# carry4985/ORB_SLAM2_MAP

Measured on AMD Instinct MI355X. Metric: frames/sec ORB extract+match (640x480, 1000 feat), higher is better.
Workload: dtype u8; 1 GPU; C2: synthetic 640x480 RGB-D stream, 1000 features, 8 levels, extract + BF-Hamming match of consecutive frames; resident_frame_pool=1024, sequences=1, parallelism=1 sequence per GPU, schedule_name=best, extraction_parts=1

## Files before the change

orb_slam2_map_amd/csrc/extractor.hip:

```cpp
#include "common.h"

#include <atomic>
#include <chrono>
#include <thread>
#include <tuple>
#include <type_traits>
#include <utility>
#include "trig_base.h"
#include "pyramid_view.h"
#include "resize_tables.h"

#include <algorithm>
#include <cfloat>
#include <cmath>
#include <cstdlib>
#include <cstring>
#include <vector>

namespace orbgpu {

constexpr int EDGE = 19;
static_assert(EDGE == RS_EDGE, "resize_tables.h builds its tables for this border");
constexpr int BORDER0 = EDGE - 3;
constexpr int HALF_PATCH = 15;
// ... 1366 lines not shown
                    my_exp += c > 1;
                    k++;
                }
            }
            if (my_exp)
                atomicAdd(&s_nexp, my_exp);
            SYNC();

            QT_MARK(14)
            if (tid_ == 0) {
                s_n = n2;
                if (n2 >= N || n2 == n)
                    s_done = 1;
                else if (phase == 1 && n2 + 3 * s_nexp > N)
                    s_phase = 2;
            }
            SYNC();
        };
        if (n <= QT_SOLO_MAX) {
            if ((tid >> 6) == 0)
                node_sections(tid & 63, 64, [] { qt_wave_sync(); }, [](int *arr, int cnt) { return wave_excl_scan(arr, cnt); });
        } else
            node_sections(tid, nt, [] { __syncthreads(); }, [&](int *arr, int cnt) { return block_excl_scan(arr, cnt, s_tmp); });
        __syncthreads();
        done_cur = s_done;
        if (done_cur == 2)
            break;
        n_cur = s_n;
        phase_cur = s_phase;
        for (int i = tid; i < n_cur * 4; i += nt)
            S.ccnt_next[i] = 0;
        __syncthreads();
        const bool count_next = done_cur == 0;
        const bool last_pass = done_cur == 1;
        unsigned long long *best_next = reinterpret_cast<unsigned long long *>(S.ccnt_next);

        QT_MARK(15)
        for (int i0 = tid; i0 - tid < nkeys; i0 += QT_ILP * nt) {
            uint32_t key[QT_ILP];
            int nd[QT_ILP], nn[QT_ILP];
#pragma unroll
            for (int u = 0; u < QT_ILP; u++) {
                const int i = min(i0 + u * nt, nkeys - 1);
                key[u] = key_at(i);
                nd[u] = node_of(i, key[u]);
            }
#pragma unroll
            for (int u = 0; u < QT_ILP; u++)
                nn[u] = S.inE[nd[u]] ? S.cpos[nd[u] * 4 + quadrant_at(key[u], midA[nd[u]])] : S.opos[nd[u]];
#pragma unroll
            for (int u = 0; u < QT_ILP; u++) {
                const bool have = i0 + u * nt < nkeys;
                if (last_pass) {
                    if (have)
                        atomicMax(&best_next[nn[u]], best_of(key[u]));
                    continue;
                }
                if (have)
                    set_node(i0 + u * nt, nn[u]);
                if (count_next)
                    count_runs(S.ccnt_next, nn[u] * 4 + quadrant_at(key[u], midB[nn[u]]), have && cntB[nn[u]] > 1);
            }
        }
        __syncthreads();
        best_done = last_pass;
        labelled = labelled || !last_pass;
        {
            int *t = S.ccnt;
            S.ccnt = S.ccnt_next;
            S.ccnt_next = t;
        }
        {
            short4 *tb = bndA; bndA = bndB; bndB = tb;
            int *tc = cntA; cntA = cntB; cntB = tc;
            uint16_t *tr = creA; creA = creB; creB = tr;
            uint32_t *tm = midA; midA = midB; midB = tm;
        }
        __syncthreads();
    }

    QT_MARK(3)
    const int n = n_cur;
    unsigned long long *best = reinterpret_cast<unsigned long long *>(S.ccnt);
    if (!best_done) {
        for (int p = tid; p < n; p += nt)
            best[p] = 0ull;
        __syncthreads();
        for (int i0 = tid; i0 < nkeys; i0 += QT_ILP * nt) {
            uint32_t key[QT_ILP];
            int nd[QT_ILP];
#pragma unroll
            for (int u = 0; u < QT_ILP; u++) {
                const int i = min(i0 + u * nt, nkeys - 1);
                key[u] = key_at(i);
                nd[u] = node_of(i, key[u]);
            }
#pragma unroll
            for (int u = 0; u < QT_ILP; u++)
                if (i0 + u * nt < nkeys)
                    atomicMax(&best[nd[u]], best_of(key[u]));
        }
    }
    __syncthreads();
    uint32_t *osel = sel + (size_t)f * sel_cap_total + g.sel_off;
    const bool ok = done_cur != 2 && n <= g.sel_cap;
    for (int p = tid; p < n && ok; p += nt) {
        const unsigned long long b = best[p];
        const uint32_t yx = (uint32_t)((0xFFFFFFFFFFull - (b & 0xFFFFFFFFFFull)) & 0xFFFFFFull);
        osel[p] = (yx << 8) | (uint32_t)((b >> 40) - 1ull);
    }
    QT_MARK(4)
    if (tid == 0)
        nsel[(size_t)f * nlevels + level] = ok ? n : -1;
}

struct KpAux {
    int x, y, level;
    float angle;
    float ca, sb;
    int plane_off, pitch;
};

__device__ __forceinline__ float fast_atan2_deg(float y, float x)
{
    const float s = (float)(180 / 3.14159265358979323846);
    const float p1 = 0.9997878412794807f * s, p3 = -0.3258083974640975f * s;
    const float p5 = 0.1555786518463281f * s, p7 = -0.04432655554792128f * s;
    const float ax = fabsf(x), ay = fabsf(y);
    float a, c, c2;
    if (ax >= ay) {
        c = ay / (ax + (float)DBL_EPSILON);
        c2 = c * c;
        a = (((p7 * c2 + p5) * c2 + p3) * c2 + p1) * c;
    } else {
        c = ax / (ay + (float)DBL_EPSILON);
        c2 = c * c;
        a = 90.f - (((p7 * c2 + p5) * c2 + p3) * c2 + p1) * c;
    }
    if (x < 0)
        a = 180.f - a;
    if (y < 0)
        a = 360.f - a;
    return a;
}

struct UMax {
    int v[16];
};

constexpr int OR_ITERS = 4;
constexpr int OR_BATCH_MIN = 32;
constexpr int PYR_BATCH_MIN = 32;

__global__ __launch_bounds__(256) void k_orient(const uint8_t *__restrict__ pyr, size_t frame_pyr,
                                                const LevelGeom *__restrict__ geom, int nlevels,
                                                const uint32_t *__restrict__ sel, int sel_cap_total,
                                                const int *__restrict__ nsel, const uint32_t *__restrict__ orw,
                                                orbgpu_keypoint *__restrict__ kps, KpAux *__restrict__ aux,
                                                int cap, int *__restrict__ n_out, int iters, Src0 s0)
{
    __shared__ uint32_t W10[4 * 16 * 9], M01[4 * 16 * 9];
    __shared__ __align__(16) uint8_t stage[8][31 * 48];
    for (int i = threadIdx.x; i < 4 * 16 * 9; i += 256) {
        W10[i] = orw[i];
        M01[i] = orw[4 * 16 * 9 + i];
    }
    __syncthreads();

    const int hl = threadIdx.x & 31;
    int bx, f;
    xcd_frame_block(bx, f);
    f = serpentine(f);
    const int *ns = nsel + (size_t)f * nlevels;
    for (int it = 0; it < iters; it++) {
    const int slot = (bx * iters + it) * 8 + (threadIdx.x >> 5);
    int level = -1, j = 0, out_off = 0, total = 0, cnt_l = 0;
    bool bad = false;
    struct {
        int plane_off, pitch, sel_off, patch;
        float scale;
    } g = {0, 0, 0, 0, 1.f};
    for (int l = 0; l < nlevels; l++) {
        const int c = ns[l];
        if (c < 0)
            bad = true;
        const int so = geom[l].sel_off;
        if (slot >= so && slot < so + geom[l].sel_cap) {
            level = l;
            j = slot - so;
            out_off = total;
            cnt_l = c;
            g.plane_off = geom[l].plane_off;
            g.pitch = geom[l].pitch;
            g.sel_off = so;
            g.patch = geom[l].patch;
            g.scale = geom[l].scale;
        }
        total += max(c, 0);
    }
    if (slot == 0 && hl == 0)
        n_out[f] = bad ? -1 - total : (total > cap ? -1 - total : total);
    if (level < 0 || bad || total > cap || j >= cnt_l)
        continue;
    const uint32_t key = sel[(size_t)f * sel_cap_total + g.sel_off + j];
    const int x = key_x(key) + BORDER0, y = key_y(key) + BORDER0;
    const bool dir0 = s0.direct != 0 && level == 0;
    const int porg = dir0 ? 0 : EDGE, ppitch = dir0 ? (int)s0.pitch : g.pitch;
    const int xl = x + porg - HALF_PATCH;
    const int a = xl & 3;
    const int v = hl - HALF_PATCH;
    int m10 = 0, m01 = 0;
    {
        const uint8_t *base = (dir0 ? s0.p + (size_t)f * s0.frame_stride : pyr + (size_t)f * frame_pyr + g.plane_off) + (xl - a);
        struct __attribute__((packed, aligned(4))) Piece {
            uint32_t d[4];
        };
        const int lim = a == 2 ? 3 : (a == 3 ? 6 : -1);
        const uint8_t *rowbase = base + rowoff(y + porg - HALF_PATCH, ppitch);
        uint4 *pl = reinterpret_cast<uint4 *>(stage[threadIdx.x >> 5]);
        Piece pc[3];
#pragma unroll
        for (int k = 0; k < 2; k++) {
            const int q = hl + 32 * k, r = q >> 1, part = q & 1;
            if (q < 62)
                pc[k] = *reinterpret_cast<const Piece *>(rowbase + rowoff(r, ppitch) + part * 16);
        }
        const int r2 = HALF_PATCH - lim + hl;
        if (hl < 2 * lim + 1)
            pc[2] = *reinterpret_cast<const Piece *>(rowbase + rowoff(r2, ppitch) + 32);
#pragma unroll
        for (int k = 0; k < 2; k++) {
            const int q = hl + 32 * k;
            if (q < 62)
                pl[3 * (q >> 1) + (q & 1)] = make_uint4(pc[k].d[0], pc[k].d[1], pc[k].d[2], pc[k].d[3]);
        }
        if (hl < 2 * lim + 1)
            pl[3 * r2 + 2] = make_uint4(pc[2].d[0], pc[2].d[1], pc[2].d[2], pc[2].d[3]);
        __builtin_amdgcn_fence(__ATOMIC_RELEASE, "wavefront");
        __builtin_amdgcn_wave_barrier();
        __builtin_amdgcn_fence(__ATOMIC_ACQUIRE, "wavefront");
        if (hl < 31) {
            const int av = v < 0 ? -v : v;
            const uint32_t *row = reinterpret_cast<const uint32_t *>(stage[threadIdx.x >> 5]) + hl * 12;
            const uint32_t *w = &W10[(a * 16 + av) * 9], *m = &M01[(a * 16 + av) * 9];
            uint32_t sw = 0, sm = 0;
#pragma unroll
            for (int q = 0; q < 9; q++) {
                const uint32_t d = row[q];
                sw = __builtin_amdgcn_udot4(d, w[q], sw, false);
                sm = __builtin_amdgcn_udot4(d, m[q], sm, false);
            }
            m10 = (int)sw - 16 * (int)sm;
            m01 = v * (int)sm;
        }
        __builtin_amdgcn_fence(__ATOMIC_RELEASE, "wavefront");
        __builtin_amdgcn_wave_barrier();
    }
#pragma unroll
    for (int off = 16; off > 0; off >>= 1) {
        m10 += __shfl_xor(m10, off, 64);
        m01 += __shfl_xor(m01, off, 64);
    }
    if (hl == 0) {
        const float angle = fast_atan2_deg((float)m01, (float)m10);
        orbgpu_keypoint kp;
        kp.x = (float)x;
        kp.y = (float)y;
        if (level != 0) {
            kp.x *= g.scale;
            kp.y *= g.scale;
        }
        kp.size = (float)g.patch;
        kp.angle = angle;
        kp.response = (float)key_resp(key);
        kp.octave = level;
        kp.class_id = -1;
        kps[(size_t)f * cap + out_off + j] = kp;
        KpAux ax;
        ax.x = x + (dir0 ? BLUR0_OX - EDGE : 0);
        ax.y = y;
        ax.level = level;
        ax.plane_off = g.plane_off;
        ax.pitch = g.pitch;
        ax.angle = angle;
        aux[(size_t)f * cap + out_off + j] = ax;
    }
    }
}
__global__ __launch_bounds__(256) void k_trig(KpAux *__restrict__ aux, const int *__restrict__ n_out, int cap, TrigTable tt)
{
    const int f = blockIdx.y;
    const int i = blockIdx.x * 256 + threadIdx.x;
    if (i >= n_out[f])
        return;
    KpAux *a = aux + (size_t)f * cap + i;
    const float factorPI = (float)(3.14159265358979323846 / 180.f);
    const float angle = a->angle * factorPI;
    float c, s;
    orbgpu_trig_device(angle, tt, &c, &s);
    a->ca = c;
    a->sb = s;
}

constexpr int BLUR_ROWS = 30;

__device__ __forceinline__ void blur_hsum(uint32_t d0, uint32_t d1, uint32_t d2, uint32_t h[4])
{
#define W4(a, b, c, d) ((uint32_t)(a) | ((uint32_t)(b) << 8) | ((uint32_t)(c) << 16) | ((uint32_t)(d) << 24))
    h[0] = __builtin_amdgcn_udot4(d1, W4(55, 49, 34, 18), __builtin_amdgcn_udot4(d0, W4(0, 18, 34, 49), 0u, false), false);
    h[1] = __builtin_amdgcn_udot4(d2, W4(18, 0, 0, 0), __builtin_amdgcn_udot4(d1, W4(49, 55, 49, 34), __builtin_amdgcn_udot4(d0, W4(0, 0, 18, 34), 0u, false), false), false);
    h[2] = __builtin_amdgcn_udot4(d2, W4(34, 18, 0, 0), __builtin_amdgcn_udot4(d1, W4(34, 49, 55, 49), __builtin_amdgcn_udot4(d0, W4(0, 0, 0, 18), 0u, false), false), false);
    h[3] = __builtin_amdgcn_udot4(d2, W4(49, 34, 18, 0), __builtin_amdgcn_udot4(d1, W4(18, 34, 49, 55), 0u, false), false);
#undef W4
}

__device__ __forceinline__ uint32_t blur_vsum(const uint32_t A[4], const uint32_t C[4], const uint32_t E[4],
                                              const uint32_t F[4])
{
    const us2 K01 = {18, 34}, K23 = {49, 55}, K45 = {49, 34}, K6 = {0, 18};
    uint32_t sv[4];
#pragma unroll
    for (int p = 0; p < 4; p++) {
        uint32_t acc = __builtin_amdgcn_udot2(__builtin_bit_cast(us2, A[p]), K01, 32768u, false);
        acc = __builtin_amdgcn_udot2(__builtin_bit_cast(us2, C[p]), K23, acc, false);
        acc = __builtin_amdgcn_udot2(__builtin_bit_cast(us2, E[p]), K45, acc, false);
        sv[p] = __builtin_amdgcn_udot2(__builtin_bit_cast(us2, F[p]), K6, acc, false);
    }
    const us2 cap = {255, 255};
    const us2 lo = __builtin_elementwise_min(__builtin_bit_cast(us2, __builtin_amdgcn_perm(sv[1], sv[0], 0x07060302u)), cap);
    const us2 hi = __builtin_elementwise_min(__builtin_bit_cast(us2, __builtin_amdgcn_perm(sv[3], sv[2], 0x07060302u)), cap);
    return __builtin_amdgcn_perm(__builtin_bit_cast(uint32_t, hi), __builtin_bit_cast(uint32_t, lo), 0x06040200u);
}

__global__ __launch_bounds__(256) void k_blur(const uint8_t *__restrict__ pyr, uint8_t *__restrict__ blur,
                                               size_t frame_pyr, const LevelGeom *__restrict__ geom, StripGeom bg, int strip0)
{
    int bx, f;
    xcd_frame_block(bx, f);
    f = serpentine(f);
    const int strip = strip0 + bx * 256 + threadIdx.x;
    if (strip >= bg.first[bg.nlevels])
        return;
    int level = 0;
#pragma unroll
    for (int l = 1; l < ORBGPU_MAX_LEVELS; l++)
        level += (l < bg.nlevels && strip >= bg.first[l]) ? 1 : 0;
    const LevelGeom g = geom[level];
    const int local = strip - bg.first[level];
    const int sy = local / bg.nsx[level], sx = local - sy * bg.nsx[level];
    const int col = (4 + 2 * sx) * 4;
    const int y0 = sy * BLUR_ROWS;
    const int rows = min(BLUR_ROWS, g.h - y0);
    const uint8_t *fsrc = pyr + (size_t)f * frame_pyr;
    uint8_t *fdst = blur + (size_t)f * frame_pyr;
    const uint32_t pitch = (uint32_t)g.pitch;
    const uint32_t src0 = (uint32_t)g.plane_off + (uint32_t)(y0 + EDGE - 3) * pitch + (uint32_t)(col - 4);
    uint32_t soff = src0 + 6u * pitch;
    uint32_t doff = (uint32_t)g.plane_off + (uint32_t)(y0 + EDGE) * pitch + (uint32_t)col;
    struct __attribute__((packed, aligned(4))) Q4 {
        uint32_t d[4];
    };
    uint32_t p0[8], p1[8], p2[8], p3[8], p4[8], p5[8], hn[8];
    Q4 nx;
#define B8_HSUM(R, Q)                                                                                        \
    {                                                                                                        \
        blur_hsum(Q.d[0], Q.d[1], Q.d[2], R);                                                                \
        blur_hsum(Q.d[1], Q.d[2], Q.d[3], R + 4);                                                            \
    }
#define B8_PAIR(P, PREV, H)                                                                                  \
    _Pragma("unroll") for (int p = 0; p < 8; p++) P[p] = __builtin_amdgcn_alignbit(H[p], PREV[p], 16);
#define B8_LOAD(P, PREV, row)                                                                                \
    {                                                                                                        \
        const Q4 q = *reinterpret_cast<const Q4 *>(fsrc + (src0 + (uint32_t)(row) * pitch));                \
        B8_HSUM(hn, q)                                                                                       \
        B8_PAIR(P, PREV, hn)                                                                                 \
    }
#define B8_STEP(A, C, E, F, k)                                                                               \
    if ((k) < rows) {                                                                                        \
        B8_HSUM(hn, nx)                                                                                      \
        B8_PAIR(F, E, hn)                                                                                    \
        soff += pitch;                                                                                       \
        if ((k) + 1 < rows)                                                                                  \
            nx = *reinterpret_cast<const Q4 *>(fsrc + soff);                                                 \
        uint2 o;                                                                                             \
        o.x = blur_vsum(A, C, E, F);                                                                         \
        o.y = blur_vsum(A + 4, C + 4, E + 4, F + 4);                                                         \
        *reinterpret_cast<uint2 *>(fdst + doff) = o;                                                         \
        doff += pitch;                                                                                       \
    }
#pragma unroll
    for (int p = 0; p < 8; p++)
        p5[p] = 0;
    B8_LOAD(p5, p5, 0) B8_LOAD(p0, p5, 1) B8_LOAD(p1, p0, 2) B8_LOAD(p2, p1, 3) B8_LOAD(p3, p2, 4) B8_LOAD(p4, p3, 5)
    nx = *reinterpret_cast<const Q4 *>(fsrc + soff);
#pragma unroll 1
    for (int k = 0; k < BLUR_ROWS; k += 6) {
        B8_STEP(p0, p2, p4, p5, k)
        B8_STEP(p1, p3, p5, p0, k + 1)
        B8_STEP(p2, p4, p0, p1, k + 2)
        B8_STEP(p3, p5, p1, p2, k + 3)
        B8_STEP(p4, p0, p2, p3, k + 4)
        B8_STEP(p5, p1, p3, p4, k + 5)
    }
#undef B8_PAIR
#undef B8_STEP
#undef B8_LOAD
#undef B8_HSUM
}

__global__ __launch_bounds__(256) void k_blur0_direct(Src0 s0, uint8_t *__restrict__ blur, size_t frame_pyr,
                                                       const LevelGeom *__restrict__ geom)
{
    int bx, f;
    xcd_frame_block(bx, f);
    f = serpentine(f);
    const LevelGeom g = geom[0];
    const int nsx = g.w >> 3;
    const int strip = bx * 256 + threadIdx.x;
    const int sy = strip / nsx, sx = strip - sy * nsx;
    const int y0 = sy * BLUR_ROWS;
    if (y0 >= g.h)
        return;
    const int rows = min(BLUR_ROWS, g.h - y0);
    const bool first = sx == 0, last = sx == nsx - 1;
    const uint8_t *fsrc = s0.p + (size_t)f * s0.frame_stride + (first ? 0 : (last ? g.w - 16 : 8 * sx - 4));
    uint8_t *fdst = blur + (size_t)f * frame_pyr;
    const uint32_t pitch = (uint32_t)g.pitch;
    uint32_t doff = (uint32_t)g.plane_off + (uint32_t)(y0 + EDGE) * pitch + (uint32_t)(8 * sx + BLUR0_OX);
    struct __attribute__((packed, aligned(4))) Q4 {
        uint32_t d[4];
    };
    struct __attribute__((packed, aligned(4))) O2 {
        uint32_t d[2];
    };
    auto fetch = [&](int y) -> Q4 {
        const int ry = y < 0 ? -y : (y >= g.h ? 2 * g.h - 2 - y : y);
        return *reinterpret_cast<const Q4 *>(fsrc + __umul24((unsigned)ry, s0.pitch));
    };
    auto window = [&](const Q4 &q) -> Q4 {
        Q4 w;
        const uint32_t left = __builtin_amdgcn_perm(q.d[1], q.d[0], 0x01020304u);
// ... 759 lines not shown
    }
    if (which == 1)
        return;
    if (e->blur_geom.first[nl] > strip0)
        L.launch(k_blur, dim3((e->blur_geom.first[nl] - strip0 + 255) / 256, batch), dim3(256), 0, pyr, blur,
                           e->frame_pyr, dg, e->blur_geom, strip0);
}

static int launch_pipeline(orbgpu_extractor *e, const uint8_t *d_gray, int batch, int w, int h, size_t stride,
                           size_t frame_stride, orbgpu_keypoint *d_kps, uint8_t *d_desc, int cap, int *d_n_out,
                           Launcher &L)
{
    hipStream_t st = L.st;
    const int nl = e->nlevels;
    const LevelGeom *dg = e->d_geom.as<LevelGeom>();
    uint8_t *pyr = e->d_pyr.as<uint8_t>();
    uint8_t *blur = e->d_blur.as<uint8_t>();
    int rc = e->d_aux.reserve(sizeof(KpAux) * (size_t)cap * batch);
    if (rc != ORBGPU_OK)
        return rc;
    const bool rec = L.graph != nullptr;
    const bool prof = !rec && e->profiling && e->prof_calls < orbgpu_extractor::PROF_SLOTS;
    if (prof && e->ev.empty()) {
        e->ev.resize((size_t)orbgpu_extractor::PROF_SLOTS * 2 * ST_COUNT, nullptr);
        for (auto &x : e->ev)
            ORBGPU_HIP_TRY(hipEventCreate(&x));
    }
    hipEvent_t *evs = prof ? &e->ev[(size_t)e->prof_calls * 2 * ST_COUNT] : nullptr;
#define BEGIN(stage, s) if (prof && (stage) == 0) ORBGPU_HIP_TRY(hipEventRecord(evs[0], s))
#define END(stage, s)                                                          \
    {                                                                          \
        if (prof)                                                              \
            ORBGPU_HIP_TRY(hipEventRecord(evs[1 + (stage)], s));               \
        if (!rec && e->stage_signal[stage])                                    \
            ORBGPU_HIP_TRY(hipEventRecord(e->stage_signal[stage], s));         \
        if (!rec && e->pipe_signal[stage])                                     \
            ORBGPU_HIP_TRY(hipEventRecord(e->pipe_signal[stage], s));          \
    }
    const bool aligned4 = stride % 4 == 0 && frame_stride % 4 == 0 && (reinterpret_cast<uintptr_t>(d_gray) & 3) == 0;
    const bool direct = e->direct0_ok && !e->no_direct0 && aligned4 && batch >= e->direct0_min_batch;
    const Src0 s0{d_gray, frame_stride, (uint32_t)stride, direct ? 1 : 0};
    e->last_src = s0;
    e->level0_materialized = !direct;
    e->borders_materialized = !e->interior_resize;
    if (e->poison_pyramid) {
        int rcp = L.memset32(pyr, e->frame_pyr * batch, 0xA5);
        if (rcp == ORBGPU_OK)
            rcp = L.memset32(blur, e->frame_pyr * batch, 0xA5);
        if (rcp != ORBGPU_OK)
            return rcp;
    }
    BEGIN(ST_PYRAMID, st);
    const bool side_blur = e->concurrent_blur && !rec;
    Launcher Ls(e->side);
    const bool early_blur0 = side_blur && direct && !e->no_early_blur0;
    if (early_blur0) {
        ORBGPU_HIP_TRY(hipEventRecord(e->ev_fork0, st));
        ORBGPU_HIP_TRY(hipStreamWaitEvent(e->side, e->ev_fork0, 0));
        if (prof)
            ORBGPU_HIP_TRY(hipEventRecord(evs[ST_COUNT + 1], e->side));
        launch_blur(e, s0, batch, Ls, 1);
    }
    {
        if (!direct) {
            int rcb = materialize_level0(e, s0, batch, L);
            if (rcb != ORBGPU_OK)
                return rcb;
        }
        for (int l = 1; l < nl; l++) {
            const LevelGeom &gl = e->geom[l];
            dim3 gr((gl.pitch / 4 + 255) / 256, gl.h + 2 * EDGE, batch);
            const int ndw_l = (gl.pitch / 4) * (gl.h + 2 * EDGE);
            const int rows = batch >= PYR_BATCH_MIN || ndw_l >= 32768 ? PYR_ROWS : ndw_l >= 16384 ? PYR_ROWS / 2 : PYR_ROWS / 4;
            dim3 grf((resize_ndw(gl.w) * ((gl.h + rows - 1) / rows) + 255) / 256, batch);
            if (gl.rs_fast) {
                const bool dir1 = direct && l == 1;
                const int r8 = batch >= PYR_BATCH_MIN ? (dir1 ? e->r8_off_direct : e->r8_off[l]) : -1;
                if (r8 >= 0) {
                    dim3 gr8((resize_n8(gl.w) * ((gl.h + PYR_ROWS - 1) / PYR_ROWS) + 255) / 256, batch);
                    const bool shr = dir1 ? e->r8_share_direct : e->r8_share[l];
                    L.launch(dir1 ? (shr ? k_resize_fast<true, true, 8, true> : k_resize_fast<true, true, 8, false>)
                                  : (shr ? k_resize_fast<true, false, 8, true> : k_resize_fast<true, false, 8, false>), gr8, dim3(256), 0, pyr,
                             e->frame_pyr, dg, l, e->d_r8item.as<ResizeStrip>(), e->d_r8sel.as<uint4>(), e->d_r8wt.as<uint4>(),
                             e->d_yrow.as<YRow>(), r8, PYR_ROWS, s0);
                    continue;
                }
                auto kern = dir1 ? (rows == PYR_ROWS ? k_resize_fast<true, true, 4> : k_resize_fast<false, true, 4>)
                                 : (rows == PYR_ROWS ? k_resize_fast<true, false, 4> : k_resize_fast<false, false, 4>);
                L.launch(kern, grf, dim3(256), 0, pyr, e->frame_pyr, dg, l, e->d_rstrip.as<ResizeStrip>(),
                                   e->d_rsel.as<uint4>(), e->d_rwt.as<uint4>(), e->d_yrow.as<YRow>(),
                                   dir1 ? e->rs_off_direct : gl.rs_off, rows, s0);
            }
            else
                L.launch(k_resize_level, gr, dim3(256), 0, pyr, e->frame_pyr, dg, l,
                                   e->d_xtab.as<XTab>(), e->d_ytab.as<YTab>());
        }
    }
    END(ST_PYRAMID, st);
    BEGIN(ST_BLUR, st);
    if (side_blur) {
        ORBGPU_HIP_TRY(hipEventRecord(e->ev_fork, st));
        ORBGPU_HIP_TRY(hipStreamWaitEvent(e->side, e->ev_fork, 0));
        if (prof && !early_blur0)
            ORBGPU_HIP_TRY(hipEventRecord(evs[ST_COUNT + 1], e->side));
        launch_blur(e, s0, batch, Ls, early_blur0 ? 2 : 0);
        if (prof)
            ORBGPU_HIP_TRY(hipEventRecord(evs[ST_COUNT + 2], e->side));
        ORBGPU_HIP_TRY(hipEventRecord(e->ev_join, e->side));
    } else
        launch_blur(e, s0, batch, L);
    END(ST_BLUR, st);
    BEGIN(ST_FAST, st);
    if (e->counters_dirty) {
        int rcm = L.memset32(e->d_cellcnt.p, e->d_cellcnt.bytes & ~(size_t)3);
        if (rcm == ORBGPU_OK)
            rcm = L.memset32(e->d_qtaux.p, e->d_qtaux.bytes & ~(size_t)3);
        if (rcm != ORBGPU_OK)
            return rcm;
    }
    e->counters_dirty = true;
    {
        const int t_ini = std::max(e->prm.ini_th_fast, 1), t_min = std::max(e->prm.min_th_fast, 1);
        const DetectGeom &dgeo = direct ? e->det_geom_direct : e->det_geom;
        const int nwaves = (dgeo.first[nl] + FD_OWN - 1) / FD_OWN;
        L.launch(e->fast_early_out ? k_fast_detect<true> : k_fast_detect<false>, dim3((nwaves + 3) / 4, batch), dim3(256), 0, pyr, e->frame_pyr, dg,
                           dgeo, e->d_ctab.as<ColumnInfo>(), e->d_cells.as<CellDesc>(), (int)e->cells.size(),
                           e->d_slots.as<uint32_t>(), e->frame_slots, e->d_cellcnt.as<int>(), std::min(t_ini, t_min),
                           t_ini, e->fast_queue_cap, s0);
    }
    END(ST_FAST, st);
    BEGIN(ST_QUADTREE, st);
    if (batch >= QT_BATCH_MIN || e->force_batch_quadtree)
        L.launch(k_quadtree<false>, dim3(batch, nl), dim3(QT_THREADS_BATCH), e->qt_lds, dg,
                           e->d_cells.as<CellDesc>(), (int)e->cells.size(), e->d_slots.as<uint32_t>(), e->frame_slots,
                           e->d_cellcnt.as<int>(), e->d_dkey.as<uint32_t>(), e->d_dnode.as<uint16_t>(),
                           e->d_sel.as<uint32_t>(), e->sel_cap_total, e->d_nsel.as<int>(), e->d_ncand.as<int>(), nl,
                           e->ncap, std::max(e->prm.ini_th_fast, 1), 0, qt_dbg(), (int *)nullptr);
    else {
        if (e->qt_prefilter)
            L.launch(k_qt_prefilter, dim3(std::min((e->max_slots_level + QT_PRE_KEYS - 1) / QT_PRE_KEYS, QT_PRE_GRID), nl, batch), dim3(256), 0, dg, (int)e->cells.size(), e->d_slots.as<uint32_t>(), e->frame_slots, e->d_cellcnt.as<int>(),
                               e->d_dkey.as<uint32_t>(), e->d_qtaux.as<int>(), std::max(e->prm.ini_th_fast, 1));
        L.launch(k_quadtree<true>, dim3(batch, nl), dim3(w * h >= QT_LARGE_PIXELS ? QT_THREADS : QT_THREADS_SMALL), e->qt_lds + (size_t)e->qt_kcap * 6, dg,
                           e->d_cells.as<CellDesc>(), (int)e->cells.size(), e->d_slots.as<uint32_t>(), e->frame_slots,
                           e->d_cellcnt.as<int>(), e->d_dkey.as<uint32_t>(), e->d_dnode.as<uint16_t>(),
                           e->d_sel.as<uint32_t>(), e->sel_cap_total, e->d_nsel.as<int>(), e->d_ncand.as<int>(), nl,
                           e->ncap, std::max(e->prm.ini_th_fast, 1), e->qt_kcap, qt_dbg(),
                           e->qt_prefilter ? e->d_qtaux.as<int>() : (int *)nullptr);
    }
    if (!rec)
        ORBGPU_HIP_TRY(hipGetLastError());
    e->counters_dirty = false;
    END(ST_QUADTREE, st);
    BEGIN(ST_ORIENT, st);
    const int or_iters = batch >= OR_BATCH_MIN ? OR_ITERS : 1;
    L.launch(k_orient, dim3((e->sel_cap_total + 8 * or_iters - 1) / (8 * or_iters), batch), dim3(256), 0, pyr, e->frame_pyr, dg, nl,
                       e->d_sel.as<uint32_t>(), e->sel_cap_total, e->d_nsel.as<int>(),
                       reinterpret_cast<const uint32_t *>(e->d_pattern.as<uint8_t>() + 1024), d_kps,
                       e->d_aux.as<KpAux>(), cap, d_n_out, or_iters, s0);
    L.launch(k_trig, dim3((std::min(cap, e->max_kp) + 255) / 256, batch), dim3(256), 0,
                       e->d_aux.as<KpAux>(), d_n_out, cap, e->trig);
    END(ST_ORIENT, st);
    BEGIN(ST_DESCRIBE, st);
    if (side_blur)
        ORBGPU_HIP_TRY(hipStreamWaitEvent(st, e->ev_join, 0));
    L.launch(k_describe, dim3((std::min(cap, e->max_kp) + 7) / 8, batch), dim3(256), 0, blur,
                       e->frame_pyr, dg, e->d_aux.as<KpAux>(), d_n_out, cap, e->d_pattern.as<int8_t>(), d_desc);
    END(ST_DESCRIBE, st);
#undef BEGIN
#undef END
    if (!rec)
        ORBGPU_HIP_TRY(hipGetLastError());
    else if (L.err != hipSuccess) {
        set_error("recording the extraction graph: %s", hipGetErrorString(L.err));
        return ORBGPU_EHIP;
    }
    if (prof)
        e->prof_calls++;
    e->last_batch = batch;
    e->last_cap = cap;
    (void)w;
    (void)h;
    return ORBGPU_OK;
}

}

namespace orbgpu {

int extractor_pyramid_view(const orbgpu_extractor *e, PyramidView *v)
{
    ORBGPU_REQUIRE(e && v, "null argument");
    memset(v, 0, sizeof(*v));
    v->device_id = e->prm.device_id;
    v->nlevels = e->nlevels;
    v->scale_factor = e->prm.scale_factor;
    v->last_batch = (int)e->geom.size() == e->nlevels ? e->last_batch : 0;
    for (int l = 0; l < e->nlevels; l++) {
        v->scale[l] = e->scale[l];
        v->inv_scale[l] = e->inv_scale[l];
        if (v->last_batch > 0) {
            const LevelGeom &g = e->geom[l];
            v->w[l] = g.w;
            v->h[l] = g.h;
            v->pitch[l] = g.pitch;
            v->plane_off[l] = g.plane_off;
        }
    }
    v->pyr = e->d_pyr.as<uint8_t>();
    v->frame_pyr = e->frame_pyr;
    v->border = EDGE;
    v->direct = v->last_batch > 0 && e->last_src.direct ? 1 : 0;
    v->l0 = v->direct ? e->last_src.p : nullptr;
    v->l0_frame_stride = v->direct ? e->last_src.frame_stride : 0;
    v->l0_pitch = v->direct ? e->last_src.pitch : 0;
    v->scratch = &e->d_stereo;
    return ORBGPU_OK;
}

}

extern "C" {

int orbgpu_extractor_create(const orbgpu_extractor_params *p, orbgpu_extractor **out)
{
    std::lock_guard<std::mutex> lifecycle(orbgpu::lifecycle_mutex());
    ORBGPU_REQUIRE(p && out, "null argument");
    ORBGPU_REQUIRE(p->nlevels >= 1 && p->nlevels <= ORBGPU_MAX_LEVELS, "nlevels must be in [1,%d]", ORBGPU_MAX_LEVELS);
    ORBGPU_REQUIRE(p->nfeatures >= 1, "nfeatures must be positive");
    ORBGPU_REQUIRE(p->scale_factor > 1.0f, "scale_factor must be > 1");
    ORBGPU_REQUIRE(p->ini_th_fast >= 0 && p->ini_th_fast <= 255 && p->min_th_fast >= 0 && p->min_th_fast <= 255,
                   "FAST thresholds must be in [0,255]");
    int rc = select_device(p->device_id);
    if (rc != ORBGPU_OK)
        return rc;
    orbgpu_extractor *e = new (std::nothrow) orbgpu_extractor();
    if (!e) {
        set_error("out of host memory");
        return ORBGPU_ENOMEM;
    }
    e->prm = *p;
    if (e->prm.max_batch < 1)
        e->prm.max_batch = 1;
    e->force_batch_quadtree = getenv("ORBGPU_DEBUG_QT_BATCH") != nullptr;
    e->qt_no_prefilter = getenv("ORBGPU_DEBUG_QT_NOPRE") != nullptr;
    if (const char *q = getenv("ORBGPU_DEBUG_QT_KEYS"))
        e->qt_keys_hook = std::max(atoi(q), 0);
    e->no_direct0 = getenv("ORBGPU_DEBUG_NO_DIRECT0") != nullptr;
    e->poison_pyramid = getenv("ORBGPU_DEBUG_POISON_PYRAMID") != nullptr;
    e->no_early_blur0 = getenv("ORBGPU_DEBUG_NO_EARLY_BLUR0") != nullptr;
    if (const char *q = getenv("ORBGPU_DEBUG_DIRECT0_MIN"))
        e->direct0_min_batch = std::max(atoi(q), 1);
    if (const char *q = getenv("ORBGPU_FAST_EARLY_OUT"))
        e->fast_early_out = atoi(q) != 0;
    e->pinned_staging = getenv("ORBGPU_DEBUG_NO_PINNED") == nullptr;
    if (getenv("ORBGPU_DEBUG_NO_GRAPH"))
        e->graph_state = -1;
    if (const char *q = getenv("ORBGPU_DEBUG_FAST_QUEUE"))
        e->fast_queue_cap = std::min(std::max(atoi(q), 0), FD_QCAP);
    e->nlevels = p->nlevels;
    build_tables(e);
    hipError_t he = hipStreamCreateWithFlags(&e->stream, hipStreamNonBlocking);
    if (he != hipSuccess) {
        set_error("hipStreamCreate: %s", hipGetErrorString(he));
        delete e;
        return ORBGPU_EHIP;
    }
    rc = trig_table_for_device(p->device_id, &e->trig);
    if (rc != ORBGPU_OK) {
        (void)hipStreamDestroy(e->stream);
        delete e;
        return rc;
    }
    *out = e;
    return ORBGPU_OK;
}

int orbgpu_extractor_destroy(orbgpu_extractor *e)
{
    std::lock_guard<std::mutex> lifecycle(orbgpu::lifecycle_mutex());
    if (!e)
        return ORBGPU_OK;
    (void)hipSetDevice(e->prm.device_id);
    (void)hipDeviceSynchronize();
    DevBuf *bufs[] = {&e->d_geom, &e->d_cells, &e->d_xtab, &e->d_ytab, &e->d_yrow, &e->d_pattern, &e->d_rstrip, &e->d_rsel,
                      &e->d_rwt, &e->d_ctab, &e->d_bcol, &e->d_pyr,
                      &e->d_blur, &e->d_slots, &e->d_cellcnt, &e->d_dkey, &e->d_dnode, &e->d_sel, &e->d_nsel,
                      &e->d_ncand, &e->d_aux, &e->d_in, &e->d_kps, &e->d_desc, &e->d_nout, &e->d_dbg, &e->d_qtaux, &e->d_stereo};
    for (DevBuf *b : bufs)
        b->release();
    for (auto &x : e->ev)
        if (x)
            (void)hipEventDestroy(x);
    if (e->graph_exec)
        (void)hipGraphExecDestroy(e->graph_exec);
    if (e->graph)
        (void)hipGraphDestroy(e->graph);
    if (e->h_pin)
        (void)hipHostFree(e->h_pin);
    if (e->stream)
        (void)hipStreamDestroy(e->stream);
    if (e->side)
        (void)hipStreamDestroy(e->side);
    if (e->ev_fork)
        (void)hipEventDestroy(e->ev_fork);
    if (e->ev_fork0)
        (void)hipEventDestroy(e->ev_fork0);
    if (e->ev_join)
        (void)hipEventDestroy(e->ev_join);
    delete e;
    return ORBGPU_OK;
}

int orbgpu_extractor_get_levels(const orbgpu_extractor *e, int32_t *n)
// ... 576 lines not shown
```

Baseline: 297,500 frames/s.

## Template orient kernel, prefetch next patch, and fuse trig into orient for batches

The orientation kernel is templated on its iteration count. Keys and level geometry are loaded up front, the weight-table loads overlap the first patch fetch, and the global load for the next keypoint's patch is issued before the current one's moments are computed. For large batches the cosine/sine computation that k_trig did is folded into k_orient, which removes one kernel launch and a read-modify-write pass over the aux array. In exchange the kernel holds more registers and adds two block-wide syncs for the trig step.

Result: no change. 299,400 frames/s, median of 6 (+0.6%).

```diff
diff --git a/orb_slam2_map_amd/csrc/extractor.hip b/orb_slam2_map_amd/csrc/extractor.hip
--- a/orb_slam2_map_amd/csrc/extractor.hip
+++ b/orb_slam2_map_amd/csrc/extractor.hip
@@ -1542,141 +1542,223 @@
 constexpr int OR_BATCH_MIN = 32;
 constexpr int PYR_BATCH_MIN = 32;
 
+template <int ITERS, bool TRIG>
 __global__ __launch_bounds__(256) void k_orient(const uint8_t *__restrict__ pyr, size_t frame_pyr,
                                                 const LevelGeom *__restrict__ geom, int nlevels,
                                                 const uint32_t *__restrict__ sel, int sel_cap_total,
                                                 const int *__restrict__ nsel, const uint32_t *__restrict__ orw,
                                                 orbgpu_keypoint *__restrict__ kps, KpAux *__restrict__ aux,
-                                                int cap, int *__restrict__ n_out, int iters, Src0 s0)
-{
-    __shared__ uint32_t W10[4 * 16 * 9], M01[4 * 16 * 9];
+                                                int cap, int *__restrict__ n_out, Src0 s0, TrigTable tt)
+{
+    constexpr int NW = 4 * 16 * 9, NWK = (NW + 255) / 256;
+    __shared__ uint32_t W10[NW], M01[NW];
     __shared__ __align__(16) uint8_t stage[8][31 * 48];
-    for (int i = threadIdx.x; i < 4 * 16 * 9; i += 256) {
-        W10[i] = orw[i];
-        M01[i] = orw[4 * 16 * 9 + i];
-    }
-    __syncthreads();
-
+    uint32_t tw[NWK], tm[NWK];
+#pragma unroll
+    for (int k = 0; k < NWK; k++) {
+        const int i = min((int)threadIdx.x + 256 * k, NW - 1);
+        tw[k] = orw[i];
+        tm[k] = orw[NW + i];
+    }
     const int hl = threadIdx.x & 31;
+    const int hw = threadIdx.x >> 5;
+    const int half = threadIdx.x & 32;
     int bx, f;
     xcd_frame_block(bx, f);
     f = serpentine(f);
+    const int slot0 = bx * (ITERS * 8) + hw;
+    uint32_t key[ITERS];
+#pragma unroll
+    for (int it = 0; it < ITERS; it++)
+        key[it] = sel[(size_t)f * sel_cap_total + min(slot0 + 8 * it, sel_cap_total - 1)];
+    const LevelGeom *gl = geom + min(hl, nlevels - 1);
+    const int gl_plane = gl->plane_off, gl_pitch = gl->pitch, gl_patch = gl->patch;
+    const float gl_scale = gl->scale;
     const int *ns = nsel + (size_t)f * nlevels;
-    for (int it = 0; it < iters; it++) {
-    const int slot = (bx * iters + it) * 8 + (threadIdx.x >> 5);
-    int level = -1, j = 0, out_off = 0, total = 0, cnt_l = 0;
+    int lv[ITERS], oi[ITERS];
+#pragma unroll
+    for (int it = 0; it < ITERS; it++) {
+        lv[it] = -1;
+        oi[it] = 0;
+    }
+    int total = 0;
     bool bad = false;
-    struct {
-        int plane_off, pitch, sel_off, patch;
-        float scale;
-    } g = {0, 0, 0, 0, 1.f};
     for (int l = 0; l < nlevels; l++) {
         const int c = ns[l];
         if (c < 0)
             bad = true;
-        const int so = geom[l].sel_off;
-        if (slot >= so && slot < so + geom[l].sel_cap) {
-            level = l;
-            j = slot - so;
-            out_off = total;
-            cnt_l = c;
-            g.plane_off = geom[l].plane_off;
-            g.pitch = geom[l].pitch;
-            g.sel_off = so;
-            g.patch = geom[l].patch;
-            g.scale = geom[l].scale;
+        const int so = geom[l].sel_off, sc = geom[l].sel_cap;
+#pragma unroll
+        for (int it = 0; it < ITERS; it++) {
+            const int j = slot0 + 8 * it - so;
+            if (j >= 0 && j < sc) {
+                lv[it] = j < c ? l : -1;
+                oi[it] = total + j;
+            }
         }
         total += max(c, 0);
     }
-    if (slot == 0 && hl == 0)
+    if (bx == 0 && threadIdx.x == 0)
         n_out[f] = bad ? -1 - total : (total > cap ? -1 - total : total);
-    if (level < 0 || bad || total > cap || j >= cnt_l)
-        continue;
-    const uint32_t key = sel[(size_t)f * sel_cap_total + g.sel_off + j];
-    const int x = key_x(key) + BORDER0, y = key_y(key) + BORDER0;
-    const bool dir0 = s0.direct != 0 && level == 0;
-    const int porg = dir0 ? 0 : EDGE, ppitch = dir0 ? (int)s0.pitch : g.pitch;
-    const int xl = x + porg - HALF_PATCH;
-    const int a = xl & 3;
-    const int v = hl - HALF_PATCH;
-    int m10 = 0, m01 = 0;
-    {
-        const uint8_t *base = (dir0 ? s0.p + (size_t)f * s0.frame_stride : pyr + (size_t)f * frame_pyr + g.plane_off) + (xl - a);
-        struct __attribute__((packed, aligned(4))) Piece {
-            uint32_t d[4];
-        };
+    if (bad || total > cap) {
+#pragma unroll
+        for (int it = 0; it < ITERS; it++)
+            lv[it] = -1;
+    }
+
+    struct __attribute__((packed, aligned(4))) Piece {
+        uint32_t d[4];
+    };
+    Piece pc[3];
+    int al[ITERS] = {};
+    auto request = [&](int it) {
+        const int level = lv[it];
+        const bool dir0 = s0.direct != 0 && level == 0;
+        const int plane_off = __shfl(gl_plane, half + level, 64), pitch = __shfl(gl_pitch, half + level, 64);
+        const int x = key_x(key[it]) + BORDER0, y = key_y(key[it]) + BORDER0;
+        const int porg = dir0 ? 0 : EDGE, ppitch = dir0 ? (int)s0.pitch : pitch;
+        const int xl = x + porg - HALF_PATCH;
+        const int a = xl & 3;
+        al[it] = a;
+        const uint8_t *base = (dir0 ? s0.p + (size_t)f * s0.frame_stride : pyr + (size_t)f * frame_pyr + plane_off) + (xl - a);
         const int lim = a == 2 ? 3 : (a == 3 ? 6 : -1);
         const uint8_t *rowbase = base + rowoff(y + porg - HALF_PATCH, ppitch);
-        uint4 *pl = reinterpret_cast<uint4 *>(stage[threadIdx.x >> 5]);
-        Piece pc[3];
 #pragma unroll
         for (int k = 0; k < 2; k++) {
             const int q = hl + 32 * k, r = q >> 1, part = q & 1;
             if (q < 62)
                 pc[k] = *reinterpret_cast<const Piece *>(rowbase + rowoff(r, ppitch) + part * 16);
         }
-        const int r2 = HALF_PATCH - lim + hl;
         if (hl < 2 * lim + 1)
-            pc[2] = *reinterpret_cast<const Piece *>(rowbase + rowoff(r2, ppitch) + 32);
-#pragma unroll
-        for (int k = 0; k < 2; k++) {
-            const int q = hl + 32 * k;
-            if (q < 62)
-                pl[3 * (q >> 1) + (q & 1)] = make_uint4(pc[k].d[0], pc[k].d[1], pc[k].d[2], pc[k].d[3]);
-        }
-        if (hl < 2 * lim + 1)
-            pl[3 * r2 + 2] = make_uint4(pc[2].d[0], pc[2].d[1], pc[2].d[2], pc[2].d[3]);
+            pc[2] = *reinterpret_cast<const Piece *>(rowbase + rowoff(HALF_PATCH - lim + hl, ppitch) + 32);
+    };
+    if (lv[0] >= 0)
+        request(0);
+#pragma unroll
+    for (int k = 0; k < NWK; k++) {
+        const int i = threadIdx.x + 256 * k;
+        if (i < NW) {
+            W10[i] = tw[k];
+            M01[i] = tm[k];
+        }
+    }
+    __syncthreads();
+
+    const int v = hl - HALF_PATCH;
+    float ang[ITERS];
+#pragma unroll
+    for (int it = 0; it < ITERS; it++) {
+        ang[it] = 0.f;
+        const bool have = lv[it] >= 0;
+        const int a = al[it];
+        if (have) {
+            uint4 *pl = reinterpret_cast<uint4 *>(stage[hw]);
+            const int lim = a == 2 ? 3 : (a == 3 ? 6 : -1);
+#pragma unroll
+            for (int k = 0; k < 2; k++) {
+                const int q = hl + 32 * k;
+                if (q < 62)
+                    pl[3 * (q >> 1) + (q & 1)] = make_uint4(pc[k].d[0], pc[k].d[1], pc[k].d[2], pc[k].d[3]);
+            }
+            if (hl < 2 * lim + 1)
+                pl[3 * (HALF_PATCH - lim + hl) + 2] = make_uint4(pc[2].d[0], pc[2].d[1], pc[2].d[2], pc[2].d[3]);
+        }
         __builtin_amdgcn_fence(__ATOMIC_RELEASE, "wavefront");
         __builtin_amdgcn_wave_barrier();
         __builtin_amdgcn_fence(__ATOMIC_ACQUIRE, "wavefront");
-        if (hl < 31) {
-            const int av = v < 0 ? -v : v;
-            const uint32_t *row = reinterpret_cast<const uint32_t *>(stage[threadIdx.x >> 5]) + hl * 12;
-            const uint32_t *w = &W10[(a * 16 + av) * 9], *m = &M01[(a * 16 + av) * 9];
-            uint32_t sw = 0, sm = 0;
-#pragma unroll
-            for (int q = 0; q < 9; q++) {
-                const uint32_t d = row[q];
-                sw = __builtin_amdgcn_udot4(d, w[q], sw, false);
-                sm = __builtin_amdgcn_udot4(d, m[q], sm, false);
+        const int nx = it + 1 < ITERS ? it + 1 : it;
+        if (nx != it && lv[nx] >= 0)
+            request(nx);
+        if (have) {
+            int m10 = 0, m01 = 0;
+            if (hl < 31) {
+                const int av = v < 0 ? -v : v;
+                const uint32_t *row = reinterpret_cast<const uint32_t *>(stage[hw]) + hl * 12;
+                const uint32_t *w = &W10[(a * 16 + av) * 9], *m = &M01[(a * 16 + av) * 9];
+                uint32_t sw = 0, sm = 0;
+#pragma unroll
+                for (int q = 0; q < 9; q++) {
+                    const uint32_t d = row[q];
+                    sw = __builtin_amdgcn_udot4(d, w[q], sw, false);
+                    sm = __builtin_amdgcn_udot4(d, m[q], sm, false);
+                }
+                m10 = (int)sw - 16 * (int)sm;
+                m01 = v * (int)sm;
             }
-            m10 = (int)sw - 16 * (int)sm;
-            m01 = v * (int)sm;
+#pragma unroll
+            for (int off = 16; off > 0; off >>= 1) {
+                m10 += __shfl_xor(m10, off, 64);
+                m01 += __shfl_xor(m01, off, 64);
+            }
+            ang[it] = fast_atan2_deg((float)m01, (float)m10);
         }
         __builtin_amdgcn_fence(__ATOMIC_RELEASE, "wavefront");
         __builtin_amdgcn_wave_barrier();
     }
-#pragma unroll
-    for (int off = 16; off > 0; off >>= 1) {
-        m10 += __shfl_xor(m10, off, 64);
-        m01 += __shfl_xor(m01, off, 64);
-    }
-    if (hl == 0) {
-        const float angle = fast_atan2_deg((float)m01, (float)m10);
+
+    uint32_t mkey = 0;
+    int mlv = -1, moi = 0;
+    float angle = 0.f;
+#pragma unroll
+    for (int it = 0; it < ITERS; it++)
+        if (hl == it) {
+            mkey = key[it];
+            mlv = lv[it];
+            moi = oi[it];
+            angle = ang[it];
+        }
+    const int src = half + max(mlv, 0);
+    const int plane_off = __shfl(gl_plane, src, 64), pitch = __shfl(gl_pitch, src, 64), patch = __shfl(gl_patch, src, 64);
+    const float scale = __shfl(gl_scale, src, 64);
+    float ca = 0.f, sb = 0.f;
+    if (TRIG) {
+        uint32_t *mine = reinterpret_cast<uint32_t *>(stage[hw]);
+        if (hl < ITERS)
+            mine[hl] = __float_as_uint(angle);
+        __syncthreads();
+        if (threadIdx.x < 8 * ITERS) {
+            const float factorPI = (float)(3.14159265358979323846 / 180.f);
+            uint32_t *slot_of = reinterpret_cast<uint32_t *>(stage[threadIdx.x / ITERS]);
+            float c, s;
+            orbgpu_trig_device(__uint_as_float(slot_of[threadIdx.x % ITERS]) * factorPI, tt, &c, &s);
+            slot_of[ITERS + 2 * (threadIdx.x % ITERS)] = __float_as_uint(c);
+            slot_of[ITERS + 2 * (threadIdx.x % ITERS) + 1] = __float_as_uint(s);
+        }
+        __syncthreads();
+        if (hl < ITERS) {
+            ca = __uint_as_float(mine[ITERS + 2 * hl]);
+            sb = __uint_as_float(mine[ITERS + 2 * hl + 1]);
+        }
+    }
+    if (mlv >= 0) {
+        const int x = key_x(mkey) + BORDER0, y = key_y(mkey) + BORDER0;
+        const bool dir0 = s0.direct != 0 && mlv == 0;
         orbgpu_keypoint kp;
         kp.x = (float)x;
         kp.y = (float)y;
-        if (level != 0) {
-            kp.x *= g.scale;
-            kp.y *= g.scale;
-        }
-        kp.size = (float)g.patch;
+        if (mlv != 0) {
+            kp.x *= scale;
+            kp.y *= scale;
+        }
+        kp.size = (float)patch;
         kp.angle = angle;
-        kp.response = (float)key_resp(key);
-        kp.octave = level;
+        kp.response = (float)key_resp(mkey);
+        kp.octave = mlv;
         kp.class_id = -1;
-        kps[(size_t)f * cap + out_off + j] = kp;
+        kps[(size_t)f * cap + moi] = kp;
         KpAux ax;
         ax.x = x + (dir0 ? BLUR0_OX - EDGE : 0);
         ax.y = y;
-        ax.level = level;
-        ax.plane_off = g.plane_off;
-        ax.pitch = g.pitch;
+        ax.level = mlv;
+        ax.plane_off = plane_off;
+        ax.pitch = pitch;
         ax.angle = angle;
-        aux[(size_t)f * cap + out_off + j] = ax;
-    }
-    }
-}
+        ax.ca = ca;
+        ax.sb = sb;
+        aux[(size_t)f * cap + moi] = ax;
+    }
+}
+
 __global__ __launch_bounds__(256) void k_trig(KpAux *__restrict__ aux, const int *__restrict__ n_out, int cap, TrigTable tt)
 {
     const int f = blockIdx.y;
@@ -2742,13 +2824,15 @@
     e->counters_dirty = false;
     END(ST_QUADTREE, st);
     BEGIN(ST_ORIENT, st);
-    const int or_iters = batch >= OR_BATCH_MIN ? OR_ITERS : 1;
-    L.launch(k_orient, dim3((e->sel_cap_total + 8 * or_iters - 1) / (8 * or_iters), batch), dim3(256), 0, pyr, e->frame_pyr, dg, nl,
+    const bool kp_batch = batch >= OR_BATCH_MIN;
+    const int or_iters = kp_batch ? OR_ITERS : 1;
+    L.launch(kp_batch ? k_orient<OR_ITERS, true> : k_orient<1, false>, dim3((e->sel_cap_total + 8 * or_iters - 1) / (8 * or_iters), batch), dim3(256), 0, pyr, e->frame_pyr, dg, nl,
                        e->d_sel.as<uint32_t>(), e->sel_cap_total, e->d_nsel.as<int>(),
                        reinterpret_cast<const uint32_t *>(e->d_pattern.as<uint8_t>() + 1024), d_kps,
-                       e->d_aux.as<KpAux>(), cap, d_n_out, or_iters, s0);
-    L.launch(k_trig, dim3((std::min(cap, e->max_kp) + 255) / 256, batch), dim3(256), 0,
-                       e->d_aux.as<KpAux>(), d_n_out, cap, e->trig);
+                       e->d_aux.as<KpAux>(), cap, d_n_out, s0, e->trig);
+    if (!kp_batch)
+        L.launch(k_trig, dim3((std::min(cap, e->max_kp) + 255) / 256, batch), dim3(256), 0,
+                           e->d_aux.as<KpAux>(), d_n_out, cap, e->trig);
     END(ST_ORIENT, st);
     BEGIN(ST_DESCRIBE, st);
     if (side_blur)
```
